# xbarin02/libdwt

Measured on AMD Instinct MI355X. Metric: Gsamples/s (= % HBM3E BW) CDF 9/7 2-D fwd float, 8192^2 5-level, higher is better.
Workload: dtype f32

## Files before the change

libdwt_amd/csrc/dwt_backend.hip:

```cpp
#include "dwt_backend.h"

namespace dwtb {

thread_local Ctx g;
thread_local char g_err[512] = "";

int fail(const char *fmt, ...)
{
	va_list ap;
	va_start(ap, fmt);
	vsnprintf(g_err, sizeof(g_err), fmt, ap);
	va_end(ap);
	return 1;
}

int launched(hipError_t e, const char *family, const char *what)
{
	g.stat_launches++;
	return e == hipSuccess ? 0 : fail("%s %s launch failed: %s", family, what, hipGetErrorString(e));
}

static bool dword_aligned(std::initializer_list<const void *> ptrs, std::initializer_list<long> strides)
{
	bool ok = true;
// ... 171 lines not shown
	HIP_TRY(hipStreamSynchronize(g.stream));
	for (size_t i = 0; i < g.prof_used; i++) {
		float ms = 0;
		HIP_TRY(hipEventElapsedTime(&ms, g.prof_events[i].first, g.prof_events[i].second));
		const int lv = g.prof_tag[i] & 15;
		g.prof_level_ms[lv] += ms;
		g.prof_level_n[lv]++;
		if (lv == 0) {
			g.prof_ms += ms;
			g.prof_launches++;
		}
	}
	g.prof_used = 0;
	return 0;
}

long ll_pitch_elems(int w) { return align_up(w, 4); }
static char *ll_band(int k) { return (char *)g.ll[k].p; }

size_t ll_band_bytes(const Geom &ge, int k, int batch, int es)
{
	return (size_t)ll_pitch_elems(ge.Wo(k + 1)) * ge.Ho(k + 1) * es * batch + 64;
}

int ensure_ll(const Geom &ge, int batch, int es)
{
	for (int k = 0; k < 2; k++) {
		if (g.ll_external) {
			if (g.ll[k].bytes < ll_band_bytes(ge, k, batch, es))
				return fail("the caller's workspace (dwt_hip_set_workspace) is too small: band %d needs %zu bytes", k, ll_band_bytes(ge, k, batch, es));
			continue;
		}
		if (grow(g.ll[k], ll_band_bytes(ge, k, batch, es)))
			return 1;
	}
	return 0;
}

bool level_fused_ok(const Call2d &c, const Geom &ge, int j)
{
	return !g.force_generic && (c.es == 4 || (c.es == 2 ? c.aligned : g.fused_d != 0)) && ge.Wi(j) == ge.Wo(j) && ge.Hi(j) == ge.Ho(j) && ge.Wo(j) >= 2 &&
		ge.Ho(j) >= 2;
}
static bool pair01_ok(const Call2d &c, const Geom &ge, int J, int batch)
{
	const int W = ge.Wo(0), H = ge.Ho(0);
	if (!g.fuse01 || g.fma || J < 2 || !level_fused_ok(c, ge, 0) || !level_fused_ok(c, ge, 1) || !fwd01_can(c.w, W, H))
		return false;
	const SweepTuning &t = g.tune;
	if (t.cpt == 4 || t.ring == 8 || (t.nt & 8) || (t.tile_pairs & 1))
		return false;
	if (g.fuse01 >= 2)
		return true;
	const long ntx = (W + 511) / 512, nty = ((H >> 1) + 63) / 64;
	return fwd01_tiles(W) * 10 <= ntx * 11 && ntx * nty * batch >= 32768;
}

static int half_level_begin(Img cur, Img dst, int Wo, int Ho, Img *fcur, Img *fdst)
{
	const long fp = align_up((long)Wo * 4, 256);
	if (grow(g.half_f32, (size_t)fp * Ho * 2))
		return 1;
	*fcur = Img{(char *)g.half_f32.p, fp, 4};
	if (launched(launch_half_frame_cvt(true, cur.p, cur.sx, fcur->p, fp, Wo, Ho, g.stream), "binary16 frame", "widening"))
		return 1;
	*fdst = *fcur;
	if (cur.p != dst.p) {
		*fdst = Img{(char *)g.half_f32.p + (size_t)fp * Ho, fp, 4};
		if (launched(launch_half_frame_cvt(true, dst.p, dst.sx, fdst->p, fp, Wo, Ho, g.stream), "binary16 frame", "widening"))
			return 1;
	}
	return 0;
}

static int half_level_end(Img fdst, Img dst, int Wo, int Ho)
{
	return launched(launch_half_frame_cvt(false, dst.p, dst.sx, fdst.p, fdst.sx, Wo, Ho, g.stream), "binary16 frame", "narrowing");
}

static int generic_level(const Call2d &c, bool inverse, Img in, Img out, int Wo, int Ho, int Wi, int Hi, int Wh, int Hh)
{
	const WaveletFacts &f = facts(c.w);
	const bool cols_first = inverse ? f.cols_inv : f.cols_fwd;
	Img lc = in, ld = out;
	if (widened(c.w) && half_level_begin(in, out, Wo, Ho, &lc, &ld))
		return 1;
	const bool dense = Wi == Wo && Hi == Ho && Wo >= 2 && Ho >= 2;
	if (dense && grow(g.stage_img, (size_t)ld.sx * Ho))
		return 1;
	for (int pass = 0; pass < 2; pass++) {
		const bool rows = cols_first != (pass == 0);
		if (f.skip1 && (rows ? Wo : Ho) <= 1)
			continue;
		const Img to = dense && pass == 0 ? Img{(char *)g.stage_img.p, ld.sx, ld.es} : ld;
		if (generic_pass(f.line_as, inverse, rows, lc, to, Wo, Ho, rows ? Ho : Wo, rows ? Wi : Hi, rows ? Wh : Hh))
			return 1;
		lc = to;
	}
	return widened(c.w) ? half_level_end(ld, out, Wo, Ho) : 0;
}

static hipError_t sweep_fwd(const Call2d &c, const FwdLevelArgs &a, const SweepTuning &t, hipStream_t s)
{
	return c.es == 8 ? launch_fwd_level_d(c.w, a, t, s)
	     : c.es == 4 ? launch_fwd_level(sweep32_wavelet(c.w), a, t, s)
	     : widened(c.w) ? launch_fwd_level_h(c.w, a, t, s)
	                    : launch_fwd_level_i16(c.w, a, t, s);
}
// ... 284 lines not shown
```

libdwt_amd/csrc/dwt_device.h:

```cpp
#pragma once
#include "dwt_kernels.h"
#include "dwt_lift.h"

#include <stdint.h>
#include <type_traits>

namespace dwt {

typedef unsigned u4 __attribute__((ext_vector_type(4)));
typedef unsigned u2 __attribute__((ext_vector_type(2)));

template <class T> static __device__ __forceinline__ T from_bits(unsigned u) { return __builtin_bit_cast(T, u); }
template <class T> static __device__ __forceinline__ unsigned to_bits(T v) { return __builtin_bit_cast(unsigned, v); }

#define DWT_END_PATH() asm volatile("; line-end forms" ::: "memory")

#define DWT_WAIT_VMCNT(n) asm volatile("s_waitcnt vmcnt(%0)" ::"n"(n) : "memory")

template <int AUX = 0>
static __device__ __forceinline__ void dma16(const void *g, void *l)
{
	__builtin_amdgcn_global_load_lds((const __attribute__((address_space(1))) void *)g,
		(__attribute__((address_space(3))) void *)l, 16, 0, AUX);
}
// ... 57 lines not shown
}

static __device__ __forceinline__ void lds_read3(unsigned a0, unsigned a1, unsigned a2, u4 &r0, u4 &r1, u4 &r2)
{
	asm volatile("ds_read_b128 %0, %3\n\tds_read_b128 %1, %4\n\tds_read_b128 %2, %5\n\ts_waitcnt lgkmcnt(0)"
		: "=&v"(r0), "=&v"(r1), "=&v"(r2)
		: "v"(a0), "v"(a1), "v"(a2)
		: "memory");
}

static __device__ __forceinline__ void lds_read4(unsigned a0, unsigned a1, unsigned a2, u4 &r0, u4 &r1, u4 &r2, u4 &r3)
{
	asm volatile("ds_read_b128 %0, %4\n\tds_read_b128 %1, %5\n\tds_read_b128 %2, %5 offset:16\n\tds_read_b128 %3, %6\n\ts_waitcnt lgkmcnt(0)"
		: "=&v"(r0), "=&v"(r1), "=&v"(r2), "=&v"(r3)
		: "v"(a0), "v"(a1), "v"(a2)
		: "memory");
}

static __device__ __forceinline__ void lds_issue3(unsigned a0, unsigned a1, unsigned a2, u4 &r0, u4 &r1, u4 &r2)
{
	asm volatile("ds_read_b128 %0, %3\n\tds_read_b128 %1, %4\n\tds_read_b128 %2, %5"
		: "=&v"(r0), "=&v"(r1), "=&v"(r2)
		: "v"(a0), "v"(a1), "v"(a2)
		: "memory");
}

template <int N>
static __device__ __forceinline__ void lds_arrived3(u4 &r0, u4 &r1, u4 &r2)
{
	asm volatile("s_waitcnt lgkmcnt(%3)" : "+v"(r0), "+v"(r1), "+v"(r2) : "n"(N) : "memory");
}

static __device__ __forceinline__ void lds_read2x3(unsigned a0, unsigned a1, unsigned a2, u2 &r0, u2 &r1, u2 &r2)
{
	asm volatile("ds_read_b64 %0, %3\n\tds_read_b64 %1, %4\n\tds_read_b64 %2, %5\n\ts_waitcnt lgkmcnt(0)"
		: "=&v"(r0), "=&v"(r1), "=&v"(r2)
		: "v"(a0), "v"(a1), "v"(a2)
		: "memory");
}

static __device__ __forceinline__ void lds_read1(unsigned a0, u4 &r0)
{
	asm volatile("ds_read_b128 %0, %1\n\ts_waitcnt lgkmcnt(0)" : "=&v"(r0) : "v"(a0) : "memory");
}

static __device__ __forceinline__ void lds_read2o(unsigned a0, unsigned a1, u4 &r0, u4 &r1, u4 &r2)
{
	asm volatile("ds_read_b128 %0, %3\n\tds_read_b128 %1, %3 offset:16\n\tds_read_b128 %2, %4\n\ts_waitcnt lgkmcnt(0)"
		: "=&v"(r0), "=&v"(r1), "=&v"(r2)
		: "v"(a0), "v"(a1)
		: "memory");
}

static __device__ __forceinline__ void lds_read2(unsigned a0, unsigned a1, u4 &r0, u4 &r1)
{
	asm volatile("ds_read_b128 %0, %2\n\tds_read_b128 %1, %3\n\ts_waitcnt lgkmcnt(0)"
		: "=&v"(r0), "=&v"(r1)
		: "v"(a0), "v"(a1)
		: "memory");
}

static __device__ __forceinline__ unsigned from_left_lane(unsigned v)
{
	return (unsigned)__builtin_amdgcn_update_dpp((int)v, (int)v, 0x138 , 0xf, 0xf, false);
}

static __device__ __forceinline__ unsigned from_right_lane(unsigned v)
{
	return (unsigned)__builtin_amdgcn_update_dpp((int)v, (int)v, 0x130 , 0xf, 0xf, false);
}

static __device__ __forceinline__ unsigned lds_offset(const void *p)
{
	return (unsigned)(uintptr_t)((__attribute__((address_space(3))) const void *)p);
}


static __device__ __forceinline__ int tile_block_id(int swz, int first = 0, int tile_blocks = 0)
{
	int b = blockIdx.x - first;
	const int nb = tile_blocks > 0 ? tile_blocks : gridDim.x - first;
	if (swz && (nb & 7) == 0)
		b = (b & 7) * (nb >> 3) + (b >> 3);
	return b;
}

static __device__ __forceinline__ void lds_write4(unsigned addr, u4 v)
{
	asm volatile("ds_write_b128 %0, %1" ::"v"(addr), "v"(v) : "memory");
}

static __device__ __forceinline__ unsigned lds_read_dword(unsigned addr)
{
	unsigned r;
	asm volatile("ds_read_b32 %0, %1\n\ts_waitcnt lgkmcnt(0)" : "=&v"(r) : "v"(addr) : "memory");
	return r;
}

static __device__ __forceinline__ void lds_write_dword(unsigned addr, unsigned v)
{
	asm volatile("ds_write_b32 %0, %1" ::"v"(addr), "v"(v) : "memory");
}

static __device__ __forceinline__ void wg_barrier_lds()
{
	asm volatile("s_waitcnt lgkmcnt(0)\n\ts_barrier" ::: "memory");
}

template <bool NTL, bool NTS>
static __device__ __forceinline__ void copy_rects_block(const CopyRects &r, int b)
{
	int k = 0;
	while (k + 1 < r.n && b >= r.first_block[k + 1])
		k++;
	if (b >= r.first_block[r.n])
		return;
	b -= r.first_block[k];
	constexpr int kRows = 8;
	constexpr int seg = 256 * 16;
	const int nbx = (r.wbytes[k] + seg - 1) / seg;
	const int bx = b % nbx, by = b / nbx;
	const unsigned x = (unsigned)bx * seg + threadIdx.x * 16;
// ... 32 lines not shown
```

libdwt_amd/csrc/dwt_sweep2d.hip:

```cpp
#include "dwt_sweep2d.h"

namespace dwt {

template <class W, bool INV>
__global__ __launch_bounds__(256) void k_line_pass(const char *__restrict__ src, char *__restrict__ dst,
	long line_stride, long elem_stride, int n_lines, int N, int hoff, int lanes_along_lines)
{
	using T = typename W::T;
	using S = typename storage_of<W>::type;
	constexpr int K = W::K;
	const int fast = blockIdx.x * blockDim.x + threadIdx.x;
	const int slow = blockIdx.y;
	const int line = lanes_along_lines ? fast : slow;
	const int k = lanes_along_lines ? slow : fast;
	const int npairs = (N + 1) >> 1;
	if (line >= n_lines || k >= npairs)
		return;
	const char *s = src + (long)line * line_stride;
	char *d = dst + (long)line * line_stride;
	auto ld = [&](int idx) { return (T) * (const S *)(s + (long)idx * elem_stride); };
	auto st = [&](int idx, T v) { *(S *)(d + (long)idx * elem_stride) = (S)v; };
	const bool il = hoff < 0;

	if (N == 1) {
// ... 26 lines not shown
}

template <class W>
static hipError_t line_pass_t(bool inverse, const void *src, void *dst, long line_stride, long elem_stride,
	int n_lines, int N, int hoff, bool lanes_along_lines, hipStream_t s)
{
	if (n_lines <= 0 || N <= 0)
		return hipSuccess;
	const int npairs = (N + 1) >> 1;
	const int fast = lanes_along_lines ? n_lines : npairs;
	const int slow = lanes_along_lines ? npairs : n_lines;
	const int bs = fast >= 256 ? 256 : 64;
	dim3 grid((fast + bs - 1) / bs, slow);
	if (inverse)
		k_line_pass<W, true><<<grid, bs, 0, s>>>((const char *)src, (char *)dst, line_stride, elem_stride, n_lines, N, hoff, lanes_along_lines);
	else
		k_line_pass<W, false><<<grid, bs, 0, s>>>((const char *)src, (char *)dst, line_stride, elem_stride, n_lines, N, hoff, lanes_along_lines);
	return hipGetLastError();
}

hipError_t launch_line_pass(Wavelet w, bool inverse, const void *src, void *dst, long line_stride, long elem_stride,
	int n_lines, int N, int hoff, bool lanes_along_lines, hipStream_t s)
{
	switch (w) {
	case kCdf97S: return line_pass_t<Cdf97S>(inverse, src, dst, line_stride, elem_stride, n_lines, N, hoff, lanes_along_lines, s);
	case kCdf53I: return line_pass_t<Cdf53I>(inverse, src, dst, line_stride, elem_stride, n_lines, N, hoff, lanes_along_lines, s);
	case kCdf53S: return line_pass_t<Cdf53S>(inverse, src, dst, line_stride, elem_stride, n_lines, N, hoff, lanes_along_lines, s);
	case kCdf97D: return line_pass_t<Cdf97D>(inverse, src, dst, line_stride, elem_stride, n_lines, N, hoff, lanes_along_lines, s);
	case kCdf53D: return line_pass_t<Cdf53D>(inverse, src, dst, line_stride, elem_stride, n_lines, N, hoff, lanes_along_lines, s);
	case kCdf97I: return line_pass_t<Cdf97I>(inverse, src, dst, line_stride, elem_stride, n_lines, N, hoff, lanes_along_lines, s);
	case kCdf53SNew: return line_pass_t<Cdf53SNew>(inverse, src, dst, line_stride, elem_stride, n_lines, N, hoff, lanes_along_lines, s);
	case kCdf97IIp: return line_pass_t<Cdf97IIp>(inverse, src, dst, line_stride, elem_stride, n_lines, N, hoff, lanes_along_lines, s);
	case kInterp53S: return line_pass_t<Interp53S>(inverse, src, dst, line_stride, elem_stride, n_lines, N, hoff, lanes_along_lines, s);
	case kCdf53I16: return line_pass_t<Cdf53I16>(inverse, src, dst, line_stride, elem_stride, n_lines, N, hoff, lanes_along_lines, s);
	case kCdf97H: break;
	case kCdf97SFma: return line_pass_t<Cdf97S>(inverse, src, dst, line_stride, elem_stride, n_lines, N, hoff, lanes_along_lines, s);
	}
	return hipErrorInvalidValue;
}

template <class W, int CPT, int RING, int NT, bool IL, bool X, bool F01 = false>
static __device__ __forceinline__ void fwd_sweep_tile(const FwdLevelArgs &a, const SweepGeom &g)
{
	static_assert(!F01 || (kIsSelEnds<W> && CPT == 8 && !IL && !X && W::K == 4 && !(NT & 8)), "the fused pair: float 9/7 by selection, Mallat");
	using T = typename W::T;
	constexpr int K = W::K;
	constexpr int kRing = RING;
	constexpr int kAhead = kRing / 2 - 1;
	constexpr int kLdAux = (NT & 2) ? 2 : 0;
	constexpr bool kNtStore = (NT & 1) != 0;
	[[maybe_unused]] constexpr bool kNtStoreLL = kNtStore && !(NT & 4);
	constexpr bool kShuffle = (NT & 8) != 0;
	constexpr int TW = 64 * CPT;
	constexpr int RS = TW + 8;
	constexpr int HK = (K + 1) & ~1;
	constexpr int NARR = CPT + 2 * HK;
	constexpr int kDmaPerIter = 2 * (CPT / 4 + 1);
	constexpr bool kPairRows = kIsSelEnds<W> && std::is_same<T, float>::value && has_coef_ends<W>::value && !std::is_base_of<Cdf97SFma, W>::value;
	extern __shared__ __attribute__((aligned(16))) char smem[];

	const int lane = threadIdx.x & 63;
	const SweepTile tile = sweep_tile<F01>(a, g, X ? g.first : 0, g.tile_blocks);
	if (!tile.live)
		return;
	if (a.pair_hi > 0 && (tile.A < a.pair_lo || tile.A >= a.pair_hi))
		return;
	const int wv = tile.wv, tx = tile.tx, A = tile.A, B = tile.B;
	[[maybe_unused]] const int ty = tile.ty;
	const int img = blockIdx.y;
	const int Wd = (a.W + 1) >> 1, Hd = (a.H + 1) >> 1;
	const int c0 = tx * (F01 ? TW - 32 : TW);
	const int warm = (F01 && A > 0) ? K : 0;
	const int n_iter = (B - A) + K + warm + (F01 ? 3 : 0);
	const int q0 = A - K / 2 - warm;

	const T *in = (const T *)a.in + (long)img * a.in_bstride;
	T *out_ll = (T *)a.out_ll + (long)img * a.ll_bstride;
	T *out_h = (T *)a.out_h + (long)img * a.h_bstride;

	char *ring = smem + (size_t)wv * kRing * RS * 4;
	const unsigned ring_off = lds_offset(ring);

	const int n_edge = min(4, c0 + TW - a.W);
	const int edge_col = kIsSelEnds<W> ? a.W - 2 - min(lane, 3) : reflect(a.W + min(lane, 3), a.W);
	const int halo_i = lane < 4 ? c0 - 4 + lane : c0 + TW + (lane & 3);
	const int halo_col = kIsSelEnds<W> ? reflect_near(halo_i, a.W) : reflect(halo_i, a.W);

	int islot = 0, rslot = 0;
	const bool tall = kIsSelEnds<W> || a.H >= 64;
	[[maybe_unused]] const bool shl = IL && a.sh.rows != nullptr;
	[[maybe_unused]] int halo_sh = -1;
	if (IL && shl)
		halo_sh = (halo_col >= c0 - 4 && halo_col < c0) ? 8 * (tx - 1) + (halo_col - (c0 - 4))
			: (halo_col >= c0 + TW && halo_col < c0 + TW + 4) ? 8 * tx + 4 + (halo_col - (c0 + TW)) : -1;
	auto issue = [&](int it) {
#pragma unroll
		for (int rr = 0; rr < 2; rr++) {
			const int ri = 2 * (q0 + it) - 1 + rr;
			const int r = tall ? reflect1(ri, a.H) : reflect(ri, a.H);
			char *lrow = ring + (size_t)(islot + rr) * RS * 4;
			const T *grow = in + (long)r * a.in_pitch;
			[[maybe_unused]] const T *hsrc = grow + halo_col;
			[[maybe_unused]] const T *rgt = nullptr;
			if (IL && shl) {
				if (r < 2 * A)
					grow = (const T *)a.sh.rows + (long)(9 * (ty - 1) + r - (2 * A - 5)) * a.sh.rows_pitch, hsrc = grow + halo_col;
				else if (r >= 2 * B)
					grow = (const T *)a.sh.rows + (long)(9 * ty + r - (2 * B - 5)) * a.sh.rows_pitch, hsrc = grow + halo_col;
				else if (r < kIlKeepTop)
					grow = (const T *)a.sh.top + (long)r * a.sh.top_pitch, hsrc = grow + halo_col;
				else {
					rgt = (const T *)a.sh.right + (long)r * a.sh.right_pitch - a.sh.right_x0;
					if (halo_sh >= 0)
						hsrc = (const T *)a.sh.cols + (long)r * a.sh.cols_pitch + halo_sh;
					else if (halo_col >= a.W - kIlKeepRight)
						hsrc = rgt + halo_col;
				}
			}
			[[maybe_unused]] const T *esrc = (IL && rgt) ? rgt + edge_col : grow + edge_col;
			const bool fix_right = IL && rgt && c0 + TW > a.W - kIlKeepRight;
			const row_rsrc_t rs = row_rsrc(grow, (unsigned)a.W * 4);
			if (kLdAux != 0 && it < K + warm && A > 0) {
#pragma unroll
				for (int i = 0; i < CPT / 4; i++)
					dma16_row<0>(rs, (unsigned)(c0 + i * 256 + lane * 4) * 4, lrow + i * 1024);
				if (fix_right && lane < kIlKeepRight)
					dma4<0>(rgt + (a.W - kIlKeepRight + lane), lrow + (a.W - kIlKeepRight - c0) * 4);
				if (lane < n_edge)
					dma4<0>(esrc, lrow + (a.W - c0) * 4);
				if (lane < 8)
					dma4<0>(IL ? hsrc : grow + halo_col, lrow + TW * 4);
			} else {
#pragma unroll
				for (int i = 0; i < CPT / 4; i++)
					dma16_row<kLdAux>(rs, (unsigned)(c0 + i * 256 + lane * 4) * 4, lrow + i * 1024);
				if (fix_right && lane < kIlKeepRight)
					dma4<0>(rgt + (a.W - kIlKeepRight + lane), lrow + (a.W - kIlKeepRight - c0) * 4);
				if (lane < n_edge)
					dma4<kLdAux>(esrc, lrow + (a.W - c0) * 4);
				if (lane < 8)
					dma4<0>(IL ? hsrc : grow + halo_col, lrow + TW * 4);
			}
		}
		islot = islot + 2 >= kRing ? 0 : islot + 2;
	};

	T st[K][CPT];
#pragma unroll
	for (int s = 0; s < K; s++)
#pragma unroll
		for (int v = 0; v < CPT; v++)
			st[s][v] = 0;

	[[maybe_unused]] unsigned hends = 0;
	[[maybe_unused]] bool h_any = false, h_simple = false;
	constexpr unsigned kCand = (1u << HK) | (1u << (HK + CPT - 1));
	if constexpr (W::kEndForms) {
		hends = end_mask<NARR>(c0 + lane * CPT - HK, a.W);
		h_any = !a.plain_ends && __builtin_amdgcn_ballot_w64(hends != 0) != 0;
		h_simple = __builtin_amdgcn_ballot_w64((hends & ~(kCand | 1u | (1u << (NARR - 1)))) != 0) == 0;
	}
	[[maybe_unused]] bool e0 = false, e1 = false;
	[[maybe_unused]] T kh[K];
	if constexpr (kIsSelEnds<W>) {
		const unsigned m = end_mask_long<NARR>(c0 + lane * CPT - HK, a.W);
		e0 = (m >> HK) & 1;
		e1 = (m >> (HK + CPT - 1)) & 1;
		sel_coefs<W, false, HK>(kh, e0, e1);
	}
	[[maybe_unused]] bool e1m = false, g0 = false, g5 = false, g7 = false, g9 = false, own0 = true, own1 = true;
	[[maybe_unused]] T st1[K][4] = {}, held[4] = {};
	if constexpr (F01) {
		e1m = c0 + lane * CPT + 3 == a.W - 1;
		const unsigned m1 = end_mask_long<12>((c0 >> 1) + lane * 4 - 4, a.W >> 1);
		g0 = (m1 >> 4) & 1;
		g5 = (m1 >> 5) & 1;
		g7 = (m1 >> 7) & 1;
		g9 = (m1 >> 9) & 1;
		const bool last_tile = tx == g.ntx - 1;
		own0 = last_tile || lane < 60;
		own1 = (tx == 0 || lane >= 1) && (last_tile || lane <= 60);
	}
	[[maybe_unused]] auto row_is_end = [&](int r) {
		if (tall || kIsSelEnds<W>)
			return r == 0 || r == a.H - 1;
		const int rr = reflect(r, a.H);
		return rr == 0 || rr == a.H - 1;
	};

	for (int it = 0; it < kAhead && it < n_iter; it++)
		issue(it);

	for (int it = 0; it < n_iter; it++) {
		if (it + kAhead < n_iter) {
			issue(it + kAhead);
			DWT_WAIT_VMCNT(kAhead * kDmaPerIter);
		} else {
			DWT_WAIT_VMCNT(0);
		}

		T row[2][CPT];
		[[maybe_unused]] T xs[2][kPairRows ? NARR : 1];
#pragma unroll
		for (int rr = 0; rr < 2; rr++) {
			const unsigned base = ring_off + (unsigned)(rslot + rr) * RS * 4;
			const unsigned own = base + lane * CPT * 4;
			const unsigned la = lane == 0 ? base + TW * 4 : own - 16;
			const unsigned ra = lane == 63 ? base + TW * 4 + 16 : own + CPT * 4;
			T x[NARR];
			u4 L4, R4, O0, O1;
			if constexpr (kShuffle) {
				u4 H4;
				const unsigned ha = base + TW * 4 + (lane == 63 ? 16 : 0);
				if constexpr (CPT == 8) {
					lds_read2o(own, ha, O0, O1, H4);
				} else {
					lds_read2(own, ha, O0, H4);
					O1 = O0;
				}
#pragma unroll
				for (int e = 0; e < 4; e++) {
					const unsigned l = from_left_lane(O1[e]);
					const unsigned r = from_right_lane(O0[e]);
					L4[e] = lane == 0 ? H4[e] : l;
					R4[e] = lane == 63 ? H4[e] : r;
				}
				if constexpr (CPT == 8) {
#pragma unroll
					for (int e = 0; e < 4; e++)
						x[HK + 4 + e] = from_bits<T>(O1[e]);
				}
			} else if constexpr (CPT == 8) {
				lds_read4(la, own, ra, L4, O0, O1, R4);
#pragma unroll
				for (int e = 0; e < 4; e++)
					x[HK + 4 + e] = from_bits<T>(O1[e]);
			} else {
				lds_read3(la, own, ra, L4, O0, R4);
			}
#pragma unroll
			for (int e = 0; e < HK; e++) {
				x[e] = from_bits<T>(L4[4 - HK + e]);
				x[HK + CPT + e] = from_bits<T>(R4[e]);
			}
#pragma unroll
			for (int e = 0; e < 4; e++)
				x[HK + e] = from_bits<T>(O0[e]);
			if constexpr (kPairRows) {
#pragma unroll
				for (int j = 0; j < NARR; j++)
					xs[rr][j] = x[j];
				continue;
			}
			if constexpr (W::kEndForms) {
				if (__builtin_expect(!h_any, 1)) {
					lift_fwd_regs<W, NARR>(x, 0u);
				} else if (h_simple) {
					DWT_END_PATH();
					lift_fwd_regs<W, NARR, kCand>(x, hends);
				} else {
					DWT_END_PATH();
					lift_fwd_regs<W, NARR>(x, hends);
				}
			} else if constexpr (kIsSelEnds<W>) {
				lift_regs_sel<W, NARR, false, HK, HK + CPT - 1>(x, e0, e1, kh);
			} else {
				lift_fwd_regs<W, NARR>(x, 0u);
			}
#pragma unroll
			for (int v = 0; v < CPT; v++)
				row[rr][v] = W::fwd_scale(v & 1, x[HK + v]);
		}

		if constexpr (kPairRows) {
			typedef float f2 __attribute__((ext_vector_type(2)));
			f2 x2[NARR];
#pragma unroll
			for (int j = 0; j < NARR; j++)
				x2[j] = f2{xs[0][j], xs[1][j]};
#pragma unroll
			for (int s_ = 0; s_ < K; s_++) {
#pragma unroll
				for (int j = s_ + 1; j <= NARR - 2 - s_; j += 2) {
					if (j == HK)
						x2[j] = x2[j] + kh[s_] * ((e0 ? f2{-0.0f, -0.0f} : x2[j - 1]) + x2[j + 1]);
					else if (j == HK + CPT - 1)
						x2[j] = x2[j] + kh[s_] * (x2[j - 1] + (e1 ? f2{-0.0f, -0.0f} : x2[j + 1]));
					else if (F01 && j == HK + 3)
						x2[j] = x2[j] + (e1m ? 2.0f * W::fk(s_) : W::fk(s_)) * (x2[j - 1] + (e1m ? f2{-0.0f, -0.0f} : x2[j + 1]));
					else
						x2[j] = x2[j] + W::fk(s_) * (x2[j - 1] + x2[j + 1]);
				}
			}
			const float ze = W::fwd_scale(0, 1.0f), zo = W::fwd_scale(1, 1.0f);
#pragma unroll
			for (int v = 0; v < CPT; v++) {
				const f2 sc = x2[HK + v] * ((v & 1) ? zo : ze);
				row[0][v] = sc[0];
				row[1][v] = sc[1];
			}
		}
		rslot = rslot + 2 >= kRing ? 0 : rslot + 2;

		[[maybe_unused]] bool vend[K] = {};
		[[maybe_unused]] bool v_any = false;
		if constexpr (W::kEndForms) {
#pragma unroll
			for (int s_ = 0; s_ < K; s_++) {
				vend[s_] = row_is_end(2 * (q0 + it) - 1 - s_);
				v_any = !a.plain_ends && (v_any || vend[s_]);
			}
		}
		T lo[CPT], hi[CPT];
		auto vertical = [&](auto mode) {
			if constexpr (kPairRows && K != 1) {
				static_assert(decltype(mode)::value == kColNone, "the paired pass has no explicit end forms");
				vertical_pairs<W, CPT>(row, st, lo, hi);
			} else
				fwd_vertical<W, decltype(mode)::value>(row, st, lo, hi, vend);
		};
		if constexpr (W::kEndForms) {
			if (__builtin_expect(v_any, 0)) {
				DWT_END_PATH();
				vertical(ColTag<kColEnds>{});
			}
			else
				vertical(ColTag<kColNone>{});
		} else if constexpr (kIsSelEnds<W>) {
			bool ve[K], any = false;
#pragma unroll
			for (int s_ = 0; s_ < K; s_++) {
				ve[s_] = row_is_end(2 * (q0 + it) - 1 - s_);
				any = any || ve[s_];
			}
			auto vertical_sel = [&]() {
				T kv[K];
#pragma unroll
				for (int s_ = 0; s_ < K; s_++)
					kv[s_] = sel_coef<W, false>(s_, ve[s_]);
				if constexpr (kPairRows && K != 1)
					vertical_pairs<W, CPT, true>(row, st, lo, hi, ve, kv);
				else
					fwd_vertical<W, kColSel>(row, st, lo, hi, ve, kv);
			};
			if constexpr (RING == 8 && has_coef_ends<W>::value)
				vertical_sel();
			else if (__builtin_expect(any, 0)) {
				DWT_END_PATH();
				vertical_sel();
			} else
				vertical(ColTag<kColNone>{});
		} else {
			vertical(ColTag<kColNone>{});
		}

		if constexpr (IL) {
			if (it >= K && (!X || A + it - K >= kIlKeepTop / 2) && a.out_step > 1) {
				const int k = A + it - K;
				const unsigned sb = (unsigned)a.out_step * 4;
				const unsigned cb = (unsigned)(c0 + lane * CPT) * sb;
				const unsigned row_bytes = (unsigned)((X ? a.W - kIlKeepRight : a.W) - 1) * sb + 4;
				const T *r0 = out_h + (long)(2 * k) * a.h_pitch;
				const row_rsrc_t d0 = row_rsrc(r0, row_bytes);
#pragma unroll
				for (int e = 0; e < CPT; e++)
					if ((e & 1) || !a.il_ll)
						store4_row<false>(d0, cb + e * sb, to_bits(lo[e]));
				if (2 * k + 1 < a.H) {
					const row_rsrc_t d1 = row_rsrc(r0 + a.h_pitch, row_bytes);
#pragma unroll
					for (int e = 0; e < CPT; e++)
						store4_row<false>(d1, cb + e * sb, to_bits(hi[e]));
				}
				if (a.il_ll) {
					const row_rsrc_t dl = row_rsrc(out_ll + (long)k * a.ll_pitch, (unsigned)(X ? (a.W - kIlKeepRight + 1) >> 1 : Wd) * 4);
#pragma unroll
					for (int e = 0; e < CPT; e += 4)
						store8_row<false>(dl, (unsigned)(c0 + lane * CPT) * 2 + e * 2, u2{to_bits(lo[e]), to_bits(lo[e + 2])});
				}
			} else
			if (it >= K && (!X || A + it - K >= kIlKeepTop / 2)) {
				const int k = A + it - K;
				const unsigned cb = (unsigned)(c0 + lane * CPT) * 4;
				const T *r0 = out_h + (long)(2 * k) * a.h_pitch;
				const unsigned row_bytes = (unsigned)(X ? a.W - kIlKeepRight : a.W) * 4;
				const row_rsrc_t d0 = row_rsrc(r0, row_bytes);
#pragma unroll
				for (int e = 0; e < CPT; e += 4) {
					const u4 v4{to_bits(lo[e]), to_bits(lo[e + 1]), to_bits(lo[e + 2]), to_bits(lo[e + 3])};
					if (a.il_ll == 2)
						store16_row<false>(d0, cb + e * 4, v4);
					else
						store16_row<kNtStore>(d0, cb + e * 4, v4);
				}
				if (2 * k + 1 < a.H) {
					const row_rsrc_t d1 = row_rsrc(r0 + a.h_pitch, row_bytes);
#pragma unroll
					for (int e = 0; e < CPT; e += 4)
						store16_row<kNtStore>(d1, cb + e * 4, u4{to_bits(hi[e]), to_bits(hi[e + 1]), to_bits(hi[e + 2]), to_bits(hi[e + 3])});
				}
				if (a.il_ll) {
					const row_rsrc_t dl = row_rsrc(out_ll + (long)k * a.ll_pitch, (unsigned)(X ? (a.W - kIlKeepRight + 1) >> 1 : Wd) * 4);
#pragma unroll
					for (int e = 0; e < CPT; e += 4)
						store8_row<false>(dl, cb / 2 + e * 2, u2{to_bits(lo[e]), to_bits(lo[e + 2])});
				}
			}
		} else
		if constexpr (F01) {
			typedef float f2 __attribute__((ext_vector_type(2)));
			const f2 nz = f2{-0.0f, -0.0f};
			const int k = q0 + it - K / 2;
			if (k >= A && k < B && own0) {
				const unsigned clb = (unsigned)((c0 + lane * CPT) >> 1) * 4;
				const T *top = out_h + (long)k * a.h_pitch, *bot = out_h + (long)(Hd + k) * a.h_pitch;
				const unsigned nb = (unsigned)Wd * 4;
				store16_row<kNtStore>(row_rsrc(top + Wd, nb), clb, u4{to_bits(lo[1]), to_bits(lo[3]), to_bits(lo[5]), to_bits(lo[7])});
				store16_row<kNtStore>(row_rsrc(bot, nb), clb, u4{to_bits(hi[0]), to_bits(hi[2]), to_bits(hi[4]), to_bits(hi[6])});
				store16_row<kNtStore>(row_rsrc(bot + Wd, nb), clb, u4{to_bits(hi[1]), to_bits(hi[3]), to_bits(hi[5]), to_bits(hi[7])});
			}
			if (it & 1) {
#pragma unroll
				for (int e = 0; e < 4; e++)
					held[e] = lo[2 * e];
			} else {
				const int q1 = k >> 1, W1 = Wd, H1 = Hd;
				f2 y[12];
#pragma unroll
				for (int e = 0; e < 4; e++) {
					const unsigned b0 = to_bits(held[e]), b1 = to_bits(lo[2 * e]);
					y[e] = f2{from_bits<T>(from_left_lane(b0)), from_bits<T>(from_left_lane(b1))};
					y[4 + e] = f2{held[e], lo[2 * e]};
					y[8 + e] = f2{from_bits<T>(from_right_lane(b0)), from_bits<T>(from_right_lane(b1))};
				}
#pragma unroll
				for (int s_ = 0; s_ < K; s_++) {
#pragma unroll
					for (int j = s_ + 1; j <= 10 - s_; j += 2) {
						if (j == 4 || j == 5 || j == 7 || j == 9) {
							const bool el = j == 4 && g0, er = j == 5 ? g5 : j == 7 ? g7 : j == 9 ? g9 : false;
							y[j] = y[j] + ((el || er) ? 2.0f * W::fk(s_) : W::fk(s_)) * ((el ? nz : y[j - 1]) + (er ? nz : y[j + 1]));
						} else
							y[j] = y[j] + W::fk(s_) * (y[j - 1] + y[j + 1]);
					}
				}
				const float ze = W::fwd_scale(0, 1.0f), zo = W::fwd_scale(1, 1.0f);
				bool vt[K], vb[K];
				T kv[K];
#pragma unroll
				for (int s_ = 0; s_ < K; s_++) {
					vt[s_] = 2 * q1 - 1 - s_ == 0;
					vb[s_] = 2 * q1 - 1 - s_ == H1 - 1;
					kv[s_] = (vt[s_] || vb[s_]) ? 2.0f * W::fk(s_) : W::fk(s_);
				}
				auto older = [&](int s_, f2 v) { return vt[s_] ? nz : v; };
				auto newer = [&](int s_, f2 v) { return vb[s_] ? nz : v; };
				T lo1[4], hi1[4];
#pragma unroll
				for (int v = 0; v < 2; v++) {
					const f2 c0v = y[4 + v] * (v ? zo : ze), c2v = y[6 + v] * (v ? zo : ze);
					const f2 ov = f2{c0v[0], c2v[0]}, ev = f2{c0v[1], c2v[1]};
					f2 s_[K], n_[K];
#pragma unroll
					for (int i = 0; i < K; i++)
						s_[i] = f2{st1[i][v], st1[i][v + 2]};
					n_[0] = ev;
					n_[1] = ov + kv[0] * (older(0, s_[0]) + newer(0, ev));
					n_[2] = s_[0] + kv[1] * (older(1, s_[1]) + newer(1, n_[1]));
					n_[3] = s_[1] + kv[2] * (older(2, s_[2]) + newer(2, n_[2]));
					const f2 s2n = s_[2] + kv[3] * (older(3, s_[3]) + newer(3, n_[3]));
					const f2 l2 = s2n * ze, h2 = n_[3] * zo;
#pragma unroll
					for (int i = 0; i < K; i++) {
						st1[i][v] = n_[i][0];
						st1[i][v + 2] = n_[i][1];
					}
					lo1[v] = l2[0];
					lo1[v + 2] = l2[1];
					hi1[v] = h2[0];
					hi1[v + 2] = h2[1];
				}
				const int k1 = q1 - K / 2;
				if (k1 >= (A >> 1) && k1 < (B >> 1) && own1) {
					const int W2 = W1 >> 1, H2 = H1 >> 1;
					const unsigned cb = (unsigned)((c0 >> 2) + lane * 2) * 4, nb = (unsigned)W2 * 4;
					const T *top = out_h + (long)k1 * a.h_pitch, *bot = out_h + (long)(H2 + k1) * a.h_pitch;
					store8_row<kNtStoreLL>(row_rsrc(out_ll + (long)k1 * a.ll_pitch, nb), cb, u2{to_bits(lo1[0]), to_bits(lo1[2])});
					store8_row<kNtStore>(row_rsrc(top + W2, nb), cb, u2{to_bits(lo1[1]), to_bits(lo1[3])});
					store8_row<kNtStore>(row_rsrc(bot, nb), cb, u2{to_bits(hi1[0]), to_bits(hi1[2])});
					store8_row<kNtStore>(row_rsrc(bot + W2, nb), cb, u2{to_bits(hi1[1]), to_bits(hi1[3])});
				}
			}
		} else
		if (it >= K) {
			const int k = A + it - K;
			const unsigned clb = (unsigned)((c0 + lane * CPT) >> 1) * 4;
			const T *top = out_h + (long)k * a.h_pitch, *bot = out_h + (long)(Hd + k) * a.h_pitch;
			const unsigned nlb = (unsigned)Wd * 4, nhb = (unsigned)(a.W >> 1) * 4;
			const row_rsrc_t dll = row_rsrc(out_ll + (long)k * a.ll_pitch, nlb), dhl = row_rsrc(top + Wd, nhb);
			const bool hrow = k < (a.H >> 1);
			if constexpr (CPT == 8) {
				store16_row<kNtStoreLL>(dll, clb, u4{to_bits(lo[0]), to_bits(lo[2]), to_bits(lo[4]), to_bits(lo[6])});
				store16_row<kNtStore>(dhl, clb, u4{to_bits(lo[1]), to_bits(lo[3]), to_bits(lo[5]), to_bits(lo[7])});
				if (hrow) {
					store16_row<kNtStore>(row_rsrc(bot, nlb), clb, u4{to_bits(hi[0]), to_bits(hi[2]), to_bits(hi[4]), to_bits(hi[6])});
					store16_row<kNtStore>(row_rsrc(bot + Wd, nhb), clb, u4{to_bits(hi[1]), to_bits(hi[3]), to_bits(hi[5]), to_bits(hi[7])});
				}
			} else {
				store8_row<kNtStoreLL>(dll, clb, u2{to_bits(lo[0]), to_bits(lo[2])});
				store8_row<kNtStore>(dhl, clb, u2{to_bits(lo[1]), to_bits(lo[3])});
				if (hrow) {
					store8_row<kNtStore>(row_rsrc(bot, nlb), clb, u2{to_bits(hi[0]), to_bits(hi[2])});
					store8_row<kNtStore>(row_rsrc(bot + Wd, nhb), clb, u2{to_bits(hi[1]), to_bits(hi[3])});
				}
			}
		}
	}
}

template <class W, int CPT, int RING, int NT, bool IL, bool X>
static __device__ __forceinline__ void fwd_sweep_any_tile(const FwdLevelArgs &a, const SweepGeom &g)
{
	if constexpr (W::kEndForms) {
		if (a.plain_ends)
			fwd_sweep_tile<PlainEnds<W>, CPT, RING, NT, IL, X>(a, g);
		else if (a.W % CPT == 0 && a.W >= 64 && a.H >= 64)
			fwd_sweep_tile<SelEnds<W>, CPT, RING, NT, IL, X>(a, g);
		else
			fwd_sweep_tile<W, CPT, RING, NT, IL, X>(a, g);
	} else
		fwd_sweep_tile<W, CPT, RING, NT, IL, X>(a, g);
}

template <class W, int CPT, int RING, int NT, bool IL = false>
__global__ __launch_bounds__(256) void k_fwd_sweep(FwdLevelArgs a, SweepGeom g)
{
// ... 88 lines not shown
	if (a.W < 2 || a.H < 2 || a.batch < 1)
		return hipErrorInvalidValue;
	const int cpt = a.interleaved ? 4 : pick_cpt(t, a.W, false);
	const int TW = 64 * cpt;
	SweepGeom g;
	g.tile_pairs = pick_tile_pairs(t, a.W, a.H, cpt, a.batch);
	g.ntx = (a.W + TW - 1) / TW;
	g.swz = t.xcd_swizzle;
	g.wave_horiz = 0;
	const int Hd = (a.H + 1) / 2;
	const int waves = sweep_waves(t);
	const int nty = (Hd + g.tile_pairs - 1) / g.tile_pairs;
	SweepTuning tt = t;
	if (tt.ring != 8 && tt.ring != 16)
		tt.ring = (g.ntx >= waves && (long)g.ntx * nty * a.batch >= ((a.interleaved && a.batch == 1) ? 512 : 3072)) ? 16 : 8;
	g.wave_horiz = tt.ring == 16;
	const dim3 grid = sweep_grid(g, nty, waves, a.batch);
	if (a.sh.rows && (!a.interleaved || a.batch != 1 || a.out_step != 1 || g.tile_pairs != a.sh.tile_pairs))
		return hipErrorInvalidValue;
	if (a.ride && a.ride_hi > a.ride_lo && (a.interleaved || a.batch != 1 || waves != 4 || tt.ring != 8 || a.temporal || (tt.nt & 8)))
		return hipErrorInvalidValue;
	if (a.interleaved) {
		if constexpr (std::is_same<W, Cdf97S>::value || std::is_same<W, Cdf53SNew>::value) {
			if (strip) {
				if (a.batch != 1 || a.W < 64 || a.H < 64)
					return hipErrorInvalidValue;
				return tt.ring == 16 ? fwd_launch_x<W, 16>(a, g, grid, waves, *strip, s) : fwd_launch_x<W, 8>(a, g, grid, waves, *strip, s);
			}
		}
		if (strip)
			return hipErrorInvalidValue;
		if constexpr (std::is_base_of<Cdf97S, W>::value || std::is_base_of<Cdf53S, W>::value) {
			if (tt.ring == 16)
				return fwd_launch<W, 4, 16, 3, true>(a, g, grid, waves, s);
			return fwd_launch<W, 4, 8, 3, true>(a, g, grid, waves, s);
		} else {
			return hipErrorInvalidValue;
		}
	}
	if (strip)
		return hipErrorInvalidValue;
	if (tt.nt_auto && (tt.nt & 12) == 4 && (size_t)a.batch * ((a.W + 1) / 2) * ((a.H + 1) / 2) * sizeof(typename W::T) >= ((size_t)1 << 30))
		tt.nt = 3;
	return cpt == 8 ? fwd_pick<W, 8>(a, g, grid, waves, tt, s) : fwd_pick<W, 4>(a, g, grid, waves, tt, s);
}

bool fwd01_can(Wavelet w, int W, int H)
{
	return Cdf97S::kEndForms && w == kCdf97S && W % 4 == 0 && H % 4 == 0 && W >= 128 && H >= 128;
}

int fwd01_tiles(int W)
{
	const int W1 = W >> 1;
	return W1 <= 256 ? 1 : (W1 - 256 + 239) / 240 + 1;
}

hipError_t launch_fwd01(const FwdLevelArgs &a, const SweepTuning &t, hipStream_t s)
{
	if (!fwd01_can(kCdf97S, a.W, a.H) || a.batch < 1 || a.interleaved || a.ride || a.pair_hi > 0 || (t.tile_pairs & 1))
		return hipErrorInvalidValue;
	const int waves = sweep_waves(t);
	const int Hd = a.H >> 1;
	SweepGeom g;
	g.ntx = fwd01_tiles(a.W);
	g.swz = t.xcd_swizzle;
	g.wave_horiz = 1;
	g.tile_pairs = t.tile_pairs;
	if (g.tile_pairs <= 0) {
		g.tile_pairs = 64;
		while (g.tile_pairs > 16 && (long)g.ntx * ((Hd + g.tile_pairs - 1) / g.tile_pairs) * a.batch < 1024)
			g.tile_pairs >>= 1;
	}
	const long tiles = (long)g.ntx * ((Hd + g.tile_pairs - 1) / g.tile_pairs);
	const dim3 grid((unsigned)((tiles + waves - 1) / waves), a.batch);
	const size_t lds = (size_t)waves * 16 * (64 * 8 + 8) * 4;
	const bool ll_nt = !(t.nt & 4) || (t.nt_auto && (size_t)a.batch * (a.W >> 2) * (a.H >> 2) * sizeof(float) >= ((size_t)1 << 30));
	if (ll_nt) {
		if (hipError_t e = allow_lds((const void *)k_fwd_sweep01<3>, lds))
			return e;
		k_fwd_sweep01<3><<<grid, 64 * waves, lds, s>>>(a, g);
	} else {
		if (hipError_t e = allow_lds((const void *)k_fwd_sweep01<7>, lds))
			return e;
		k_fwd_sweep01<7><<<grid, 64 * waves, lds, s>>>(a, g);
	}
	return hipGetLastError();
}

bool sweep_ride_ok(const SweepTuning &t, int W, int H, int batch, bool inverse)
{
	if (batch != 1 || W < 2 || H < 2 || !(t.waves >= 1 && t.waves <= 4 ? t.waves == 4 : true) || (t.nt & 8))
		return false;
	if (inverse)
		return t.ring_inv != 16;
	if (t.ring == 16)
		return false;
	if (t.ring == 8)
		return true;
	const int cpt = pick_cpt(t, W, false);
	const int tp = pick_tile_pairs(t, W, H, cpt, 1);
	const long ntx = (W + 64 * cpt - 1) / (64 * cpt), nty = ((H + 1) / 2 + tp - 1) / tp;
	return !(ntx >= 4 && ntx * nty >= 3072);
}

int il_sweep_tile_pairs(const SweepTuning &t, int W, int H, bool inverse)
{
	return pick_tile_pairs(t, W, H, 4, 1, inverse, true);
}

hipError_t launch_fwd_level(Wavelet w, const FwdLevelArgs &a, const SweepTuning &t, hipStream_t s, const IlStripArgs *strip)
{
	if (strip && w != kCdf97S && w != kCdf53SNew)
		return hipErrorInvalidValue;
	switch (w) {
	case kCdf97S: return fwd_level_t<Cdf97S>(a, t, s, strip);
	case kCdf53I: return fwd_level_t<Cdf53I>(a, t, s);
	case kCdf53S: return fwd_level_t<Cdf53S>(a, t, s);
	case kCdf97I: return fwd_level_t<Cdf97I>(a, t, s);
	case kCdf97SFma: return fwd_level_t<Cdf97SFma>(a, t, s);
	case kCdf53SNew: return a.interleaved ? fwd_level_t<Cdf53SNew>(a, t, s, strip) : hipErrorInvalidValue;
	case kInterp53S: return a.interleaved ? hipErrorInvalidValue : fwd_level_t<Interp53S>(a, t, s);
	default: break;
	}
	return hipErrorInvalidValue;
}

}
```

Baseline: 598.5.

## Replace overlapping fused level-0/1 tiles with wider halo and phantom-column lifting

The fused level 0+1 sweep previously overlapped neighbouring tiles by 32 columns and masked ownership of edge lanes. It now uses non-overlapping 512-column tiles with a 16-column halo on each side. Each lane group recomputes the missing neighbour level-0 low-pass columns ("phantom" columns) from the halo through horizontal and vertical lifting, and feeds them into the level-1 horizontal step through DPP lane exchange. This removes redundant recompute and re-reading of overlapped columns, so fewer tiles are launched and the fused path is chosen more often. The cost is extra halo loads, extra LDS per row, and extra per-lane arithmetic for the phantom columns.

```diff
diff --git a/libdwt_amd/csrc/dwt_backend.hip b/libdwt_amd/csrc/dwt_backend.hip
--- a/libdwt_amd/csrc/dwt_backend.hip
+++ b/libdwt_amd/csrc/dwt_backend.hip
@@ -247,8 +247,8 @@
 		return false;
 	if (g.fuse01 >= 2)
 		return true;
-	const long ntx = (W + 511) / 512, nty = ((H >> 1) + 63) / 64;
-	return fwd01_tiles(W) * 10 <= ntx * 11 && ntx * nty * batch >= 32768;
+	const long ntx = fwd01_tiles(W), nty = ((H >> 1) + 63) / 64;
+	return ntx * nty * batch >= 32768;
 }
 
 static int half_level_begin(Img cur, Img dst, int Wo, int Ho, Img *fcur, Img *fdst)
diff --git a/libdwt_amd/csrc/dwt_device.h b/libdwt_amd/csrc/dwt_device.h
--- a/libdwt_amd/csrc/dwt_device.h
+++ b/libdwt_amd/csrc/dwt_device.h
@@ -133,6 +133,20 @@
 		: "memory");
 }
 
+static __device__ __forceinline__ void lds_issue_win9x2(unsigned a0, unsigned a1, u4 &p0, u4 &p1, unsigned &p8, u4 &q0, u4 &q1, unsigned &q8)
+{
+	asm volatile("ds_read2_b64 %0, %6 offset1:1\n\tds_read2_b64 %1, %6 offset0:2 offset1:3\n\tds_read_b32 %2, %6 offset:32\n\t"
+				 "ds_read2_b64 %3, %7 offset1:1\n\tds_read2_b64 %4, %7 offset0:2 offset1:3\n\tds_read_b32 %5, %7 offset:32"
+		: "=&v"(p0), "=&v"(p1), "=&v"(p8), "=&v"(q0), "=&v"(q1), "=&v"(q8)
+		: "v"(a0), "v"(a1)
+		: "memory");
+}
+
+static __device__ __forceinline__ void lds_arrived_win9x2(u4 &p0, u4 &p1, unsigned &p8, u4 &q0, u4 &q1, unsigned &q8)
+{
+	asm volatile("s_waitcnt lgkmcnt(0)" : "+v"(p0), "+v"(p1), "+v"(p8), "+v"(q0), "+v"(q1), "+v"(q8) : : "memory");
+}
+
 static __device__ __forceinline__ void lds_read2(unsigned a0, unsigned a1, u4 &r0, u4 &r1)
 {
 	asm volatile("ds_read_b128 %0, %2\n\tds_read_b128 %1, %3\n\ts_waitcnt lgkmcnt(0)"
@@ -149,6 +163,26 @@
 static __device__ __forceinline__ unsigned from_right_lane(unsigned v)
 {
 	return (unsigned)__builtin_amdgcn_update_dpp((int)v, (int)v, 0x130 , 0xf, 0xf, false);
+}
+
+static __device__ __forceinline__ unsigned quad_lane(unsigned v, int e)
+{
+	switch (e) {
+	case 0: return (unsigned)__builtin_amdgcn_update_dpp((int)v, (int)v, 0x00, 0xf, 0xf, false);
+	case 1: return (unsigned)__builtin_amdgcn_update_dpp((int)v, (int)v, 0x55, 0xf, 0xf, false);
+	case 2: return (unsigned)__builtin_amdgcn_update_dpp((int)v, (int)v, 0xaa, 0xf, 0xf, false);
+	default: return (unsigned)__builtin_amdgcn_update_dpp((int)v, (int)v, 0xff, 0xf, 0xf, false);
+	}
+}
+
+static __device__ __forceinline__ unsigned from_left_lane(unsigned v, unsigned first)
+{
+	return (unsigned)__builtin_amdgcn_update_dpp((int)first, (int)v, 0x138 , 0xf, 0xf, false);
+}
+
+static __device__ __forceinline__ unsigned from_right_lane(unsigned v, unsigned last)
+{
+	return (unsigned)__builtin_amdgcn_update_dpp((int)last, (int)v, 0x130 , 0xf, 0xf, false);
 }
 
 static __device__ __forceinline__ unsigned lds_offset(const void *p)
diff --git a/libdwt_amd/csrc/dwt_sweep2d.hip b/libdwt_amd/csrc/dwt_sweep2d.hip
--- a/libdwt_amd/csrc/dwt_sweep2d.hip
+++ b/libdwt_amd/csrc/dwt_sweep2d.hip
@@ -102,7 +102,10 @@
 	[[maybe_unused]] constexpr bool kNtStoreLL = kNtStore && !(NT & 4);
 	constexpr bool kShuffle = (NT & 8) != 0;
 	constexpr int TW = 64 * CPT;
-	constexpr int RS = TW + 8;
+	constexpr int kHalo = F01 ? 16 : 4;
+	constexpr int RS = TW + 2 * kHalo;
+	constexpr int kHaloLanes = 2 * kHalo;
+	constexpr int kHaloL = F01 ? 8 : 0, kHaloR = F01 ? kHalo + 4 : 4;
 	constexpr int HK = (K + 1) & ~1;
 	constexpr int NARR = CPT + 2 * HK;
 	constexpr int kDmaPerIter = 2 * (CPT / 4 + 1);
@@ -119,7 +122,7 @@
 	[[maybe_unused]] const int ty = tile.ty;
 	const int img = blockIdx.y;
 	const int Wd = (a.W + 1) >> 1, Hd = (a.H + 1) >> 1;
-	const int c0 = tx * (F01 ? TW - 32 : TW);
+	const int c0 = tx * TW;
 	const int warm = (F01 && A > 0) ? K : 0;
 	const int n_iter = (B - A) + K + warm + (F01 ? 3 : 0);
 	const int q0 = A - K / 2 - warm;
@@ -133,7 +136,7 @@
 
 	const int n_edge = min(4, c0 + TW - a.W);
 	const int edge_col = kIsSelEnds<W> ? a.W - 2 - min(lane, 3) : reflect(a.W + min(lane, 3), a.W);
-	const int halo_i = lane < 4 ? c0 - 4 + lane : c0 + TW + (lane & 3);
+	const int halo_i = F01 ? (lane < 16 ? c0 - 12 + lane : c0 + TW - 4 + (lane & 15)) : lane < 4 ? c0 - 4 + lane : c0 + TW + (lane & 3);
 	const int halo_col = kIsSelEnds<W> ? reflect_near(halo_i, a.W) : reflect(halo_i, a.W);
 
 	int islot = 0, rslot = 0;
@@ -178,7 +181,7 @@
 					dma4<0>(rgt + (a.W - kIlKeepRight + lane), lrow + (a.W - kIlKeepRight - c0) * 4);
 				if (lane < n_edge)
 					dma4<0>(esrc, lrow + (a.W - c0) * 4);
-				if (lane < 8)
+				if (lane < kHaloLanes)
 					dma4<0>(IL ? hsrc : grow + halo_col, lrow + TW * 4);
 			} else {
 #pragma unroll
@@ -188,7 +191,7 @@
 					dma4<0>(rgt + (a.W - kIlKeepRight + lane), lrow + (a.W - kIlKeepRight - c0) * 4);
 				if (lane < n_edge)
 					dma4<kLdAux>(esrc, lrow + (a.W - c0) * 4);
-				if (lane < 8)
+				if (lane < kHaloLanes)
 					dma4<0>(IL ? hsrc : grow + halo_col, lrow + TW * 4);
 			}
 		}
@@ -218,8 +221,10 @@
 		e1 = (m >> (HK + CPT - 1)) & 1;
 		sel_coefs<W, false, HK>(kh, e0, e1);
 	}
-	[[maybe_unused]] bool e1m = false, g0 = false, g5 = false, g7 = false, g9 = false, own0 = true, own1 = true;
-	[[maybe_unused]] T st1[K][4] = {}, held[4] = {};
+	[[maybe_unused]] bool e1m = false, g0 = false, g5 = false, g7 = false, g9 = false, f5 = false, f7 = false;
+	[[maybe_unused]] T st1[K][4] = {}, held[4] = {}, stp[K] = {}, heldp = 0, lop = 0;
+	[[maybe_unused]] unsigned pwin = 0;
+	[[maybe_unused]] T kp[3] = {};
 	if constexpr (F01) {
 		e1m = c0 + lane * CPT + 3 == a.W - 1;
 		const unsigned m1 = end_mask_long<12>((c0 >> 1) + lane * 4 - 4, a.W >> 1);
@@ -227,9 +232,15 @@
 		g5 = (m1 >> 5) & 1;
 		g7 = (m1 >> 7) & 1;
 		g9 = (m1 >> 9) & 1;
-		const bool last_tile = tx == g.ntx - 1;
-		own0 = last_tile || lane < 60;
-		own1 = (tx == 0 || lane >= 1) && (last_tile || lane <= 60);
+		const int p = lane & 7;
+		const int pe = p < 4 ? c0 - 8 + 2 * p : c0 + TW + 2 * (p - 4);
+		pwin = (unsigned)(p < 4 ? TW + 2 * p : TW + kHalo + 2 * (p - 4)) * 4;
+		const unsigned mp = end_mask_long<9>(pe - 4, a.W);
+		f5 = (mp >> 5) & 1;
+		f7 = (mp >> 7) & 1;
+		kp[0] = f5 ? 2.0f * W::fk(0) : W::fk(0);
+		kp[1] = f5 ? 2.0f * W::fk(2) : W::fk(2);
+		kp[2] = f7 ? 2.0f * W::fk(0) : W::fk(0);
 	}
 	[[maybe_unused]] auto row_is_end = [&](int r) {
 		if (tall || kIsSelEnds<W>)
@@ -251,12 +262,19 @@
 
 		T row[2][CPT];
 		[[maybe_unused]] T xs[2][kPairRows ? NARR : 1];
+		[[maybe_unused]] u4 pw[2][2];
+		[[maybe_unused]] unsigned pw8[2];
+		[[maybe_unused]] T rowp[2] = {};
+		if constexpr (F01) {
+			const unsigned pa = ring_off + (unsigned)rslot * RS * 4 + pwin;
+			lds_issue_win9x2(pa, pa + RS * 4, pw[0][0], pw[0][1], pw8[0], pw[1][0], pw[1][1], pw8[1]);
+		}
 #pragma unroll
 		for (int rr = 0; rr < 2; rr++) {
 			const unsigned base = ring_off + (unsigned)(rslot + rr) * RS * 4;
 			const unsigned own = base + lane * CPT * 4;
-			const unsigned la = lane == 0 ? base + TW * 4 : own - 16;
-			const unsigned ra = lane == 63 ? base + TW * 4 + 16 : own + CPT * 4;
+			const unsigned la = lane == 0 ? base + (TW + kHaloL) * 4 : own - 16;
+			const unsigned ra = lane == 63 ? base + (TW + kHaloR) * 4 : own + CPT * 4;
 			T x[NARR];
 			u4 L4, R4, O0, O1;
 			if constexpr (kShuffle) {
@@ -324,6 +342,30 @@
 
 		if constexpr (kPairRows) {
 			typedef float f2 __attribute__((ext_vector_type(2)));
+			if constexpr (F01) {
+				const f2 nz = f2{-0.0f, -0.0f};
+				lds_arrived_win9x2(pw[0][0], pw[0][1], pw8[0], pw[1][0], pw[1][1], pw8[1]);
+				f2 w2[9];
+#pragma unroll
+				for (int j = 0; j < 8; j++)
+					w2[j] = f2{from_bits<T>(pw[0][j >> 2][j & 3]), from_bits<T>(pw[1][j >> 2][j & 3])};
+				w2[8] = f2{from_bits<T>(pw8[0]), from_bits<T>(pw8[1])};
+#pragma unroll
+				for (int s_ = 0; s_ < K; s_++) {
+#pragma unroll
+					for (int j = s_ + 1; j <= 7 - s_; j += 2) {
+						if (j == 5)
+							w2[j] = w2[j] + kp[s_ >> 1] * (w2[j - 1] + (f5 ? nz : w2[j + 1]));
+						else if (j == 7)
+							w2[j] = w2[j] + kp[2] * (w2[j - 1] + (f7 ? nz : w2[j + 1]));
+						else
+							w2[j] = w2[j] + W::fk(s_) * (w2[j - 1] + w2[j + 1]);
+					}
+				}
+				const f2 sc = w2[4] * W::fwd_scale(0, 1.0f);
+				rowp[0] = sc[0];
+				rowp[1] = sc[1];
+			}
 			f2 x2[NARR];
 #pragma unroll
 			for (int j = 0; j < NARR; j++)
@@ -383,11 +425,28 @@
 				ve[s_] = row_is_end(2 * (q0 + it) - 1 - s_);
 				any = any || ve[s_];
 			}
+			[[maybe_unused]] auto vertical_phantom = [&](auto sel, const T *kv) {
+				if constexpr (F01) {
+					T n[K + 1];
+					n[0] = rowp[1];
+#pragma unroll
+					for (int s_ = 0; s_ < K; s_++) {
+						const bool e = decltype(sel)::value && ve[s_];
+						n[s_ + 1] = (s_ ? stp[s_ - 1] : rowp[0]) + (decltype(sel)::value ? kv[s_] : W::fk(s_)) * ((e ? T(-0.0) : stp[s_]) + n[s_]);
+					}
+					lop = n[K] * W::fwd_scale(0, 1.0f);
+#pragma unroll
+					for (int s_ = 0; s_ < K; s_++)
+						stp[s_] = n[s_];
+				}
+			};
 			auto vertical_sel = [&]() {
 				T kv[K];
 #pragma unroll
 				for (int s_ = 0; s_ < K; s_++)
 					kv[s_] = sel_coef<W, false>(s_, ve[s_]);
+				if constexpr (F01)
+					vertical_phantom(std::true_type{}, kv);
 				if constexpr (kPairRows && K != 1)
 					vertical_pairs<W, CPT, true>(row, st, lo, hi, ve, kv);
 				else
@@ -398,8 +457,11 @@
 			else if (__builtin_expect(any, 0)) {
 				DWT_END_PATH();
 				vertical_sel();
-			} else
+			} else {
 				vertical(ColTag<kColNone>{});
+				if constexpr (F01)
+					vertical_phantom(std::false_type{}, nullptr);
+			}
 		} else {
 			vertical(ColTag<kColNone>{});
 		}
@@ -461,7 +523,7 @@
 			typedef float f2 __attribute__((ext_vector_type(2)));
 			const f2 nz = f2{-0.0f, -0.0f};
 			const int k = q0 + it - K / 2;
-			if (k >= A && k < B && own0) {
+			if (k >= A && k < B) {
 				const unsigned clb = (unsigned)((c0 + lane * CPT) >> 1) * 4;
 				const T *top = out_h + (long)k * a.h_pitch, *bot = out_h + (long)(Hd + k) * a.h_pitch;
 				const unsigned nb = (unsigned)Wd * 4;
@@ -473,15 +535,18 @@
 #pragma unroll
 				for (int e = 0; e < 4; e++)
 					held[e] = lo[2 * e];
+				heldp = lop;
 			} else {
 				const int q1 = k >> 1, W1 = Wd, H1 = Hd;
 				f2 y[12];
+				const unsigned pb0 = to_bits(heldp), pb1 = to_bits(lop);
 #pragma unroll
 				for (int e = 0; e < 4; e++) {
 					const unsigned b0 = to_bits(held[e]), b1 = to_bits(lo[2 * e]);
-					y[e] = f2{from_bits<T>(from_left_lane(b0)), from_bits<T>(from_left_lane(b1))};
+					const unsigned q0e = quad_lane(pb0, e), q1e = quad_lane(pb1, e);
+					y[e] = f2{from_bits<T>(from_left_lane(b0, q0e)), from_bits<T>(from_left_lane(b1, q1e))};
 					y[4 + e] = f2{held[e], lo[2 * e]};
-					y[8 + e] = f2{from_bits<T>(from_right_lane(b0)), from_bits<T>(from_right_lane(b1))};
+					y[8 + e] = f2{from_bits<T>(from_right_lane(b0, q0e)), from_bits<T>(from_right_lane(b1, q1e))};
 				}
 #pragma unroll
 				for (int s_ = 0; s_ < K; s_++) {
@@ -531,7 +596,7 @@
 					hi1[v + 2] = h2[1];
 				}
 				const int k1 = q1 - K / 2;
-				if (k1 >= (A >> 1) && k1 < (B >> 1) && own1) {
+				if (k1 >= (A >> 1) && k1 < (B >> 1)) {
 					const int W2 = W1 >> 1, H2 = H1 >> 1;
 					const unsigned cb = (unsigned)((c0 >> 2) + lane * 2) * 4, nb = (unsigned)W2 * 4;
 					const T *top = out_h + (long)k1 * a.h_pitch, *bot = out_h + (long)(H2 + k1) * a.h_pitch;
@@ -726,8 +791,7 @@
 
 int fwd01_tiles(int W)
 {
-	const int W1 = W >> 1;
-	return W1 <= 256 ? 1 : (W1 - 256 + 239) / 240 + 1;
+	return (W + 511) / 512;
 }
 
 hipError_t launch_fwd01(const FwdLevelArgs &a, const SweepTuning &t, hipStream_t s)
@@ -748,7 +812,7 @@
 	}
 	const long tiles = (long)g.ntx * ((Hd + g.tile_pairs - 1) / g.tile_pairs);
 	const dim3 grid((unsigned)((tiles + waves - 1) / waves), a.batch);
-	const size_t lds = (size_t)waves * 16 * (64 * 8 + 8) * 4;
+	const size_t lds = (size_t)waves * 16 * (64 * 8 + 32) * 4;
 	const bool ll_nt = !(t.nt & 4) || (t.nt_auto && (size_t)a.batch * (a.W >> 2) * (a.H >> 2) * sizeof(float) >= ((size_t)1 << 30));
 	if (ll_nt) {
 		if (hipError_t e = allow_lds((const void *)k_fwd_sweep01<3>, lds))
```

Result: faster. 614.2, median of 6 (+2.6%).
